# zj15001/PNP_ADMM_CNC_MRI

Measured on AMD Instinct MI355X. Metric: ADMM iterations/sec on 256x256 complex64 slices (batch=512), higher is better.
Workload: dtype f32

## Files before the change

pnp_admm_cnc_mri_amd/csrc/kernels_slice256.hip:

```cpp
#include "engine_host.h"
#include "fused_layout.h"
#include "slice_layout.h"
#include <math.h>
#include <stdio.h>
#include <stdlib.h>
#include <vector>

#ifndef SLICE_EARLY
#define SLICE_EARLY 1
#endif
#ifndef SLICE_PRIOSWAP
#define SLICE_PRIOSWAP 1
#endif
#ifndef SLICE_PRIOMASK
#define SLICE_PRIOMASK 6
#endif
#ifndef SLICE_YH_AUX
#define SLICE_YH_AUX 0
#endif
#ifndef SLICE_ST_AUX
#define SLICE_ST_AUX 0
#endif
#ifndef SLICE_PF
#define SLICE_PF 3
#endif

namespace pnp {

__device__ c32 g_tws[256];

struct SliceArgs {
    float* z;
    float* w;
    float* x;
    const c32* Yh;
    const uint32_t* Mh;
    const c32* Ys;
    const uint32_t* Ms;
    int first, B, iters;
    int slice_xor;
    int flip;
    int state_stride;
    int yh_stride;
    float scale, c;
    ProxParams prox;
    long long* prof;
};

constexpr int RP = 18;
constexpr int REGION = 16 * RP;
constexpr int WREG = 4 * REGION;
constexpr int SL_YS = SL_BUF + REGION;
constexpr int SL_LDS = SL_YS + 256 + 32;
static_assert(SL_WAVES * WREG <= SL_BUF, "wave regions must fit in the buffer they alias");

__device__ __forceinline__ void wave_sync() {
    __builtin_amdgcn_fence(__ATOMIC_RELEASE, "wavefront");
    __builtin_amdgcn_wave_barrier();
    __builtin_amdgcn_fence(__ATOMIC_ACQUIRE, "wavefront");
#ifdef SLICE_SYNC_SCHED_BARRIER
    __builtin_amdgcn_sched_barrier(0);
#endif
}

__device__ __forceinline__ void prio_set(int wv, int set) {
#if SLICE_PRIOSWAP
    const bool older_high = (SLICE_PRIOMASK >> set) & 1;
    if (set == 0 || (((SLICE_PRIOMASK >> set) ^ (SLICE_PRIOMASK >> (set - 1))) & 1)) {
        asm volatile("" : "+s"(wv));
        if ((wv < 4) == older_high) __builtin_amdgcn_s_setprio(1); else __builtin_amdgcn_s_setprio(0);
    }
#endif
}

__device__ __forceinline__ int opaque(int v) {
    asm volatile("" : "+v"(v));
    return v;
}
typedef unsigned int u32x4 __attribute__((ext_vector_type(4)));
typedef unsigned int u32x2 __attribute__((ext_vector_type(2)));
typedef __amdgpu_buffer_rsrc_t bufrsrc;
__device__ __forceinline__ bufrsrc make_rsrc(const void* base, unsigned bytes) {
    return __builtin_amdgcn_make_buffer_rsrc(const_cast<void*>(base), 0, (int)bytes, 0x00020000);
}
__device__ __forceinline__ void ld4(bufrsrc r, int voff, int soff, float (&v)[4]) {
    const u32x4 q = __builtin_amdgcn_raw_buffer_load_b128(r, voff, soff, 16);
    v[0] = __uint_as_float(q.x); v[1] = __uint_as_float(q.y); v[2] = __uint_as_float(q.z); v[3] = __uint_as_float(q.w);
}
__device__ __forceinline__ void st4(bufrsrc r, int voff, int soff, const float (&v)[4]) {
    u32x4 q;
    q.x = __float_as_uint(v[0]); q.y = __float_as_uint(v[1]); q.z = __float_as_uint(v[2]); q.w = __float_as_uint(v[3]);
    __builtin_amdgcn_raw_buffer_store_b128(q, r, voff + soff, 0, SLICE_ST_AUX);
}
__device__ __forceinline__ c32 ldc(bufrsrc r, int voff, int soff) {
    const u32x2 q = __builtin_amdgcn_raw_buffer_load_b64(r, voff, soff, 0);
    return mk<float>(__uint_as_float(q.x), __uint_as_float(q.y));
}
struct SliceBufs {
    bufrsrc z, w, x;
    bufrsrc yh, mh, ys, ms;
};

__device__ __forceinline__ void pin(c32& v) { asm volatile("" : "+v"(v.x), "+v"(v.y)); }
__device__ __forceinline__ void mem_fence_compiler() { asm volatile("" ::: "memory"); }

__device__ __forceinline__ float dpp_lane_xor1(float v) {
    return __int_as_float(__builtin_amdgcn_mov_dpp(__float_as_int(v), 0xB1 , 0xF, 0xF, true));
}
__device__ __forceinline__ c32 dpp_lane_xor1(c32 v) { return mk<float>(dpp_lane_xor1(v.x), dpp_lane_xor1(v.y)); }

__device__ __forceinline__ float sub_partner(float a, float b) {
    float r;
    asm("v_subrev_f32_dpp %0, %1, %2 quad_perm:[1,0,3,2] row_mask:0xf bank_mask:0xf bound_ctrl:1" : "=v"(r) : "v"(b), "v"(a));
    return r;
}
__device__ __forceinline__ float add_partner(float a, float b) {
    float r;
    asm("v_add_f32_dpp %0, %1, %2 quad_perm:[1,0,3,2] row_mask:0xf bank_mask:0xf bound_ctrl:1" : "=v"(r) : "v"(b), "v"(a));
    return r;
}

__device__ __forceinline__ float abs_plus(float a, float w) {
    float r;
    asm("v_add_f32_e64 %0, |%1|, %2" : "=v"(r) : "v"(a), "v"(w));
    return r;
}

__device__ __forceinline__ f2 sub2(f2 a, f2 b) {
    f2 r;
    asm("v_pk_add_f32 %0, %1, %2 neg_lo:[0,1] neg_hi:[0,1]" : "=v"(r) : "v"(a), "v"(b));
    return r;
}


template <bool INV>
__device__ __forceinline__ void group_fft256(c32 (&ac)[16], const c32* twl, c32* region, int t) {
    typedef float f4 __attribute__((ext_vector_type(4)));
    const f4* tw4 = reinterpret_cast<const f4*>(twl + RP * t);
    f2* reg2 = reinterpret_cast<f2*>(region);
    f2 a[16];
#pragma unroll
    for (int k = 0; k < 16; ++k) a[k] = to2(ac[k]);
    dft16_pk<INV>(a);
    mem_fence_compiler();
#pragma unroll
    for (int m = 0; m < 4; ++m) {
        const f4 q = tw4[m];
        if (m) a[2 * m] = tmul_v<INV>(a[2 * m], k2(q.x, q.y));
        a[2 * m + 1] = tmul_v<INV>(a[2 * m + 1], k2(q.z, q.w));
    }
    mem_fence_compiler();
#pragma unroll
    for (int m = 4; m < 8; ++m) {
        const f4 q = tw4[m];
        a[2 * m] = tmul_v<INV>(a[2 * m], k2(q.x, q.y));
        a[2 * m + 1] = tmul_v<INV>(a[2 * m + 1], k2(q.z, q.w));
    }
#pragma unroll
    for (int k = 0; k < 16; ++k) reg2[k * RP + t] = a[k];
    wave_sync();
    const f4* row4 = reinterpret_cast<const f4*>(reg2 + t * RP);
#pragma unroll
    for (int m = 0; m < 8; ++m) {
        const f4 q = row4[m];
        a[2 * m] = k2(q.x, q.y);
        a[2 * m + 1] = k2(q.z, q.w);
    }
    wave_sync();
    dft16_pk<INV>(a);
#pragma unroll
    for (int k = 0; k < 16; ++k) ac[k] = from2(a[k]);
}

struct RowLoads {
    float z[8][4], w[8][4];
};
__device__ __forceinline__ int row_set_offset(int set, int wv) { return (32 * set + 4 * wv) * 2048; }
constexpr int ROW_QSTRIDE = 256;

template <int PROX, bool HAS_INV, int Q0, int Q1>
__device__ __forceinline__ void issue_row_loads(const SliceBufs& b, RowLoads& L, int soff, int voff, int qbase = 0) {
#pragma unroll
    for (int q = qbase + Q0; q < qbase + Q1; ++q) {
        const int vo = voff + ROW_QSTRIDE * q, so = soff;
        if (PROX == 3) {
            ld4(b.w, vo, so, L.w[q]);
        } else if (PROX != 0 || !HAS_INV) {
            ld4(b.z, vo, so, L.z[q]);
            ld4(b.w, vo, so, L.w[q]);
        }
    }
}

__device__ __forceinline__ f2 clamp2(f2 a, float c) {
    return k2(__builtin_amdgcn_fmed3f(a.x, -c, c), __builtin_amdgcn_fmed3f(a.y, -c, c));
}
__device__ __forceinline__ f2 fma2(f2 a, f2 b, f2 c) { return __builtin_elementwise_fma(a, b, c); }
__device__ __forceinline__ f2 splat(float v) { return k2(v, v); }
template <int PROX>
__device__ __forceinline__ void prox_pair(f2 u, f2& z, f2& w, const ProxParams& pc) {
    if (PROX == 2) {
        const f2 cz = clamp2(z, pc.ib);
        const f2 t = fma2(splat(pc.c1), z, fma2(splat(pc.c2), u, splat(pc.c3) * cz));
        z = t - clamp2(t, pc.thr);
    } else {
        z = u - clamp2(u, pc.thr);
    }
    w = u - z;
}

template <bool HAS_INV, int PROX, bool HAS_FWD>
__device__ __forceinline__ void pointwise_q(const SliceBufs& b, const ProxParams& pc, int u_first, bool last,
                                            c32& a0, c32& a1, const float (&z_)[4], const float (&w_)[4], int vs) {
    f2 z[2] = {k2(z_[0], z_[1]), k2(z_[2], z_[3])}, w[2] = {k2(w_[0], w_[1]), k2(w_[2], w_[3])};
#define SL_X_PLUS(a_, w_) (HAS_INV ? k2(abs_plus((a_).x, (w_).x), abs_plus((a_).y, (w_).y)) : (w_))
#define SL_ST4(buf, v) { const float q_[4] = {v[0].x, v[0].y, v[1].x, v[1].y}; st4(buf, vs, 0, q_); }
    if (PROX == 3) {
        f2 u[2];
#pragma unroll
        for (int jj = 0; jj < 2; ++jj) {
            if (!u_first) {
                asm volatile("");
                w[jj] = w[jj] - (w[jj] - clamp2(w[jj], pc.thr));
            }
            u[jj] = SL_X_PLUS(jj ? a1 : a0, w[jj]);
            z[jj] = u[jj] - clamp2(u[jj], pc.thr);
            w[jj] = u[jj] - z[jj];
        }
        if (!last) {
            SL_ST4(b.w, u);
        } else {
            SL_ST4(b.z, z);
            SL_ST4(b.w, w);
        }
    }
    if (PROX == 1 || PROX == 2) {
#pragma unroll
        for (int jj = 0; jj < 2; ++jj) prox_pair<PROX>(SL_X_PLUS(jj ? a1 : a0, w[jj]), z[jj], w[jj], pc);
        SL_ST4(b.z, z);
        SL_ST4(b.w, w);
    }
#undef SL_ST4
#undef SL_X_PLUS
    if (HAS_FWD) {
        const f2 v0 = sub2(z[0], w[0]), v1 = sub2(z[1], w[1]);
        a0 = from2(v0);
        a1 = from2(v1);
    }
}

__device__ __forceinline__ void store_x_natural(const SliceBufs& b, const c32 (&a)[16], c32* wreg, int set, int wv, int lane) {
    const int g = lane >> 4, t = lane & 15;
    c32* region = wreg + g * REGION;
#pragma unroll
    for (int j = 0; j < 16; ++j) region[t + 16 * j] = mk<float>(fabsf(a[j].x), fabsf(a[j].y));
    wave_sync();
#pragma unroll
    for (int i = 0; i < 4; ++i) {
        const c32* cell = wreg + i * REGION + 4 * lane;
        const float4 c01 = *reinterpret_cast<const float4*>(cell);
        const float4 c23 = *reinterpret_cast<const float4*>(cell + 2);
        const int vs = 16 * lane + (2 * (32 * set + 4 * wv + i)) * 1024;
        const float xa[4] = {c01.x, c01.z, c23.x, c23.z}, xb[4] = {c01.y, c01.w, c23.y, c23.w};
        st4(b.x, vs, 0, xa);
        st4(b.x, vs + 1024, 0, xb);
    }
    wave_sync();
}

#ifndef SLICE_L1_PF
#define SLICE_L1_PF 8
#endif
template <int PROX> constexpr int row_pf() { return (PROX == 3) ? SLICE_L1_PF : SLICE_PF; }
template <int PROX, bool HAS_INV>
__device__ __forceinline__ void row_phase_prefetch(const SliceBufs& b, RowLoads& L, int wv, int lane) {
    issue_row_loads<PROX, HAS_INV, 0, row_pf<PROX>()>(b, L, row_set_offset(0, wv), 2048 * (lane >> 4) + 16 * (lane & 15));
}
template <bool HAS_INV, int PROX, bool HAS_FWD, bool PRELOADED = false>
__device__ __forceinline__ void row_phase(const SliceBufs& b, const ProxParams& pc, int u_first, bool last, c32 (&F)[SL_SETS][16],
                                          c32* wreg, const c32* twl, int wv, int lane, RowLoads* pre = nullptr) {
    const int g = lane >> 4, t = lane & 15;
    c32* region = wreg + g * REGION;
    const int voff = 2048 * g + 16 * t;
    constexpr int PF = row_pf<PROX>();
    RowLoads L;
    if (PRELOADED) L = *pre;
    else issue_row_loads<PROX, HAS_INV, 0, PF>(b, L, row_set_offset(0, wv), voff);
#pragma unroll
    for (int set = 0; set < SL_SETS; ++set) {
        c32 (&a)[16] = F[set];
        prio_set(wv, set);
        const int soff = row_set_offset(set, wv);
        if (HAS_INV) {
            group_fft256<true>(a, twl, region, t);
        }
        if (HAS_INV && last) store_x_natural(b, a, wreg, set, wv, lane);
        const int vs = voff + soff;
#pragma unroll
        for (int q = 0; q < 8; ++q) {
            if (q + PF < 8) issue_row_loads<PROX, HAS_INV, 0, 1>(b, L, soff, voff, q + PF);
            pointwise_q<HAS_INV, PROX, HAS_FWD>(b, pc, u_first, last, a[2 * q], a[2 * q + 1], L.z[q], L.w[q], vs + ROW_QSTRIDE * q);
        }
        if (set + 1 < SL_SETS) issue_row_loads<PROX, HAS_INV, 0, PF>(b, L, row_set_offset(set + 1, wv), voff);
        if (HAS_FWD) {
            group_fft256<false>(a, twl, region, t);
        }
    }
}

#define SL_PASS0_REGS(X, t)                                                                       \
    X(0, 0, (t)) X(1, 1, (t) + 16) X(2, 2, (t) + 32) X(3, 3, (t) + 48)                              \
    X(12, 8, ((t) ? SL_M + 64 - (t) : SL_M))                                                      \
    X(13, 13, SL_M + 48 - (t)) X(14, 14, SL_M + 32 - (t)) X(15, 15, SL_M + 16 - (t))
#define SL_PASS1_REGS(X, t)                                                                       \
    X(4, 4, (t)) X(5, 5, (t) + 16) X(6, 6, (t) + 32) X(7, 7, (t) + 48)                              \
    X(8, 12, ((t) ? SL_M + 64 - (t) : SL_M))                                                      \
    X(9, 9, SL_M + 48 - (t)) X(10, 10, SL_M + 32 - (t)) X(11, 11, SL_M + 16 - (t))

__device__ __forceinline__ void lds_put(c32* p, c32 v, bool swapped) {
    float* f = reinterpret_cast<float*>(p);
    if (swapped) { f[0] = v.y; f[1] = v.x; } else { *p = v; }
}
__device__ __forceinline__ c32 lds_get(const c32* p, bool swapped) {
    const float* f = reinterpret_cast<const float*>(p);
    return swapped ? mk<float>(f[1], f[0]) : *p;
}
template <int P>
__device__ __forceinline__ void t_store_rows(const c32 (&F)[16], c32* rp, int t) {
#define SL_T1_STORE(ja, jb, slot) { lds_put(rp + (slot), t ? F[ja] : F[jb], (ja) >= 8); }
    if (P == 0) { SL_PASS0_REGS(SL_T1_STORE, t) } else { SL_PASS1_REGS(SL_T1_STORE, t) }
#undef SL_T1_STORE
}
template <int P>
__device__ __forceinline__ void t_load_rows(c32 (&F)[16], const c32* rp, int t) {
#define SL_T2_LOAD(ja, jb, slot) { F[ja] = lds_get(rp + (slot), (ja) >= 8); }
    if (P == 0) { SL_PASS0_REGS(SL_T2_LOAD, t) } else { SL_PASS1_REGS(SL_T2_LOAD, t) }
#undef SL_T2_LOAD
    if (P == 1) {
        const c32 a0 = F[8];
        F[8] = t ? a0 : F[12];
        F[12] = t ? F[12] : a0;
    }
}

template <bool MAYBE_PACKED>
__device__ __forceinline__ void t1_read_col(c32 (&Gs)[16], const c32* buf, int off, int odd, bool packed) {
    int off_hi = off + 64 * SL_P;
    asm volatile("" : "+v"(off_hi));
    const c32 *col = buf + off, *col_hi = buf + off_hi;
#pragma unroll
    for (int jb = 0; jb < 16; jb += 8) {
        c32 own[8];
#pragma unroll
        for (int k = 0; k < 8; ++k) own[k] = jb ? col_hi[8 * k * SL_P] : col[8 * k * SL_P];
#pragma unroll
        for (int k = 0; k < 8; ++k) {
            c32 v = mk<float>(add_partner(own[k].x, own[k].y), sub_partner(own[k].y, own[k].x));
            if (MAYBE_PACKED) {
                const float oy = dpp_lane_xor1(own[k].y);
                const c32 raw = mk<float>(odd ? oy : own[k].x, odd ? own[k].x : oy);
                v = packed ? raw : v;
            }
            Gs[jb + k] = v;
            pin(Gs[jb + k]);
        }
    }
}
template <int P>
__device__ __forceinline__ void t1_pass(const c32 (&F)[SL_SETS][16], c32 (&G)[SL_SETS][16], c32* buf, int wv, int lane) {
    const int g = lane >> 4, t = lane & 15;
#pragma unroll
    for (int set = 0; set < SL_SETS; ++set) t_store_rows<P>(F[set], buf + (32 * set + 4 * wv + g) * SL_P, t);
    __syncthreads();
#pragma unroll
    for (int h = 0; h < 2; ++h) {
        const int cc = 32 * h + 4 * wv + g, odd = t & 1;
        const int off = (t >> 1) * SL_P + cc + (odd ? SL_M : 0);
        if (P == 0 && h == 0 && wv == 0) t1_read_col<true>(G[2 * P + h], buf, off, odd, cc == 0);
        else t1_read_col<false>(G[2 * P + h], buf, off, odd, false);
    }
    __syncthreads();
}

template <bool MAYBE_PACKED>
__device__ __forceinline__ void t2_write_col(const c32 (&Gs)[16], c32* buf, int off, int odd, bool packed) {
    int off_hi = off + 64 * SL_P;
    asm volatile("" : "+v"(off_hi));
    c32 *col = buf + off, *col_hi = buf + off_hi;
#pragma unroll
    for (int j = 0; j < 16; ++j) {
        const c32 own = Gs[j];
        c32 v = mk<float>(sub_partner(own.x, own.y), add_partner(own.y, own.x));
        if (MAYBE_PACKED) {
            const c32 other = dpp_lane_xor1(own);
            const c32 raw = mk<float>(odd ? own.y : own.x, odd ? other.y : other.x);
            v = packed ? raw : v;
        }
        if (j < 8) col[8 * j * SL_P] = v; else col_hi[8 * (j - 8) * SL_P] = v;
    }
}
template <int P>
__device__ __forceinline__ void t2_pass(const c32 (&G)[SL_SETS][16], c32 (&F)[SL_SETS][16], c32* buf, int wv, int lane) {
    const int g = lane >> 4, t = lane & 15;
#pragma unroll
    for (int h = 0; h < 2; ++h) {
        const int cc = 32 * h + 4 * wv + g, odd = t & 1;
        const int off = (t >> 1) * SL_P + cc + (odd ? SL_M : 0);
        if (P == 0 && h == 0 && wv == 0) t2_write_col<true>(G[2 * P + h], buf, off, odd, cc == 0);
        else t2_write_col<false>(G[2 * P + h], buf, off, odd, false);
    }
    __syncthreads();
#pragma unroll
    for (int set = 0; set < SL_SETS; ++set) t_load_rows<P>(F[set], buf + (32 * set + 4 * wv + g) * SL_P, t);
    __syncthreads();
}

struct ColLoads {
    c32 yh[16];
    uint32_t code;
};
__device__ __forceinline__ void issue_col_loads(const SliceBufs& b, ColLoads& Y, int set, int wv, int lane) {
    const int ybase = (set * 8 + wv) * 8192;
    Y.code = __builtin_amdgcn_raw_buffer_load_b32(b.mh, 4 * lane, (set * 8 + wv) * 64 * 4, 0);
#pragma unroll
    for (int jp = 0; jp < 8; ++jp) {
        const u32x4 q = __builtin_amdgcn_raw_buffer_load_b128(b.yh, 16 * lane + 1024 * (jp & 3), ybase + 4096 * (jp >> 2), SLICE_YH_AUX);
        Y.yh[2 * jp] = mk<float>(__uint_as_float(q.x), __uint_as_float(q.y));
        Y.yh[2 * jp + 1] = mk<float>(__uint_as_float(q.z), __uint_as_float(q.w));
    }
}

__device__ __forceinline__ float code_byte(unsigned m, int byte) {
    float r;
    if (byte == 0) asm("v_cvt_f32_ubyte0 %0, %1" : "=v"(r) : "v"(m));
    else if (byte == 1) asm("v_cvt_f32_ubyte1 %0, %1" : "=v"(r) : "v"(m));
    else if (byte == 2) asm("v_cvt_f32_ubyte2 %0, %1" : "=v"(r) : "v"(m));
    else asm("v_cvt_f32_ubyte3 %0, %1" : "=v"(r) : "v"(m));
    return r;
}
__device__ __forceinline__ void blend_set(c32 (&a)[16], const c32 (&yh)[16], unsigned code, float cs, float chs, float os) {
    const unsigned m[4] = {code & 0x03030303u, (code >> 2) & 0x03030303u, (code >> 4) & 0x03030303u, (code >> 6) & 0x03030303u};
#pragma unroll
    for (int j = 0; j < 16; j += 2) {
        const f2 cf = k2(code_byte(m[j & 3], j >> 2), code_byte(m[(j & 3) + 1], j >> 2));
        const f2 A2 = fma2(splat(-chs), cf, splat(os));
        a[j] = from2(fma2(A2.xx, to2(a[j]), splat(cs) * to2(yh[j])));
        a[j + 1] = from2(fma2(A2.yy, to2(a[j + 1]), splat(cs) * to2(yh[j + 1])));
    }
}

__device__ __forceinline__ void col_phase(const SliceBufs& b, float cdc, float scale, c32 (&G)[SL_SETS][16], c32* wreg, c32* ysl, const c32* twl, int wv, int lane) {
    const int g = lane >> 4, t = lane & 15;
    c32* region = wreg + g * REGION;
    const float cs = cdc * scale, chs = 0.5f * cdc * scale;
    ColLoads Y;
    issue_col_loads(b, Y, 0, wv, lane);
    if (wv == 0) {
        __builtin_amdgcn_raw_ptr_buffer_load_lds(b.ys, ysl, 16, 16 * lane, 0, 0, 0);
        __builtin_amdgcn_raw_ptr_buffer_load_lds(b.ys, ysl + 128, 16, 16 * lane, 1024, 0, 0);
        __builtin_amdgcn_raw_ptr_buffer_load_lds(b.ms, ysl + 256, 4, 4 * lane, 0, 0, 0);
    }
#pragma unroll
    for (int set = 0; set < SL_SETS; ++set) {
        c32 (&a)[16] = G[set];
        prio_set(wv, set);
        group_fft256<false>(a, twl, region, t);
        if (set == 0 && wv == 0 && g == 0) {
#pragma unroll
            for (int j = 0; j < 16; ++j) region[t + 16 * j] = a[j];
            region[256 + t] = a[0];
            wave_sync();
            const uint32_t code_b = reinterpret_cast<const uint32_t*>(ysl + 256)[t];
            const c32* mirror = region + (16 - t);
            const unsigned ma[4] = {Y.code & 0x03030303u, (Y.code >> 2) & 0x03030303u, (Y.code >> 4) & 0x03030303u, (Y.code >> 6) & 0x03030303u};
            const unsigned mb[4] = {code_b & 0x03030303u, (code_b >> 2) & 0x03030303u, (code_b >> 4) & 0x03030303u, (code_b >> 6) & 0x03030303u};
#pragma unroll
            for (int j = 0; j < 16; ++j) {
                const c32 gm = mirror[16 * (15 - j)];
                const c32 A = blend_scaled_f(unpack_a(a[j], gm), Y.yh[j], code_byte(ma[j & 3], j >> 2), cs, chs, scale);
                const c32 Bv = blend_scaled_f(unpack_b(a[j], gm), ysl[t + 16 * j], code_byte(mb[j & 3], j >> 2), cs, chs, scale);
                a[j] = repack_p(A, Bv);
            }
            wave_sync();
        } else {
            blend_set(a, Y.yh, Y.code, cs, 0.5f * chs, 0.5f * scale);
        }
        if (set + 1 < SL_SETS) issue_col_loads(b, Y, set + 1, wv, lane);
        group_fft256<true>(a, twl, region, t);
    }
}

template <int PROX>
__global__ __launch_bounds__(512) void k_slice(SliceArgs p) {
    __shared__ __attribute__((aligned(16))) c32 lds[SL_LDS];
    const int tid = threadIdx.x, lane = tid & 63;
    const int wv = __builtin_amdgcn_readfirstlane(tid >> 6);
    c32* twl = lds + SL_BUF;
    if (tid < 256) twl[RP * (tid >> 4) + (tid & 15)] = g_tws[((tid >> 4) * (tid & 15)) & 255];
    c32* wreg = lds + wv * WREG;
    __syncthreads();
    for (int sb = blockIdx.x; sb < p.B; sb += gridDim.x) {
        const int sx = ((sb ^ p.slice_xor) < p.B) ? (sb ^ p.slice_xor) : sb;
        const int slice = p.first + (p.flip ? p.B - 1 - sx : sx);
        const size_t so = (size_t)slice * p.state_stride;
        SliceBufs b;
        b.z = make_rsrc(p.z + so, 65536 * 4); b.w = make_rsrc(p.w + so, 65536 * 4); b.x = make_rsrc(p.x + (size_t)slice * 65536, 65536 * 4);
        b.yh = make_rsrc(p.Yh + (size_t)slice * p.yh_stride, YH3_SLICE * 8); b.mh = make_rsrc(p.Mh + (size_t)slice * MH3_SLICE, MH3_SLICE * 4);
        b.ys = make_rsrc(p.Ys + (size_t)slice * 256, 256 * 8); b.ms = make_rsrc(p.Ms + (size_t)slice * 16, 16 * 4);
        c32 F[SL_SETS][16];
#ifdef SLICE_PROF
        long long* prof = (p.prof && tid == 0 && sb == (int)blockIdx.x) ? p.prof + (size_t)slice * (2 + 6 * p.iters) : nullptr;
#define SL_STAMP() if (prof) *prof++ = wall_clock64()
#else
#define SL_STAMP()
#endif
        SL_STAMP();
        row_phase<false, 0, true>(b, p.prox, 1, false, F, wreg, twl, wv, opaque(lane));
        SL_STAMP();
        for (int it = 0; it < p.iters; ++it) {
            c32 G[SL_SETS][16];
            __syncthreads();
            SL_STAMP();
            t1_pass<0>(F, G, lds, wv, opaque(lane));
            t1_pass<1>(F, G, lds, wv, opaque(lane));
#ifdef SLICE_PROF_CLOCK
            if (prof) *prof++ = (long long)__builtin_readcyclecounter();
#else
            SL_STAMP();
#endif
            col_phase(b, p.c, p.scale, G, wreg, lds + SL_YS, twl, wv, opaque(lane));
            SL_STAMP();
            __syncthreads();
            SL_STAMP();
            t2_pass<0>(G, F, lds, wv, opaque(lane));
#if SLICE_EARLY
            RowLoads L0;
            row_phase_prefetch<PROX, true>(b, L0, wv, opaque(lane));
#endif
            t2_pass<1>(G, F, lds, wv, opaque(lane));
            SL_STAMP();
            const int u_first = (it == 0);
#if SLICE_EARLY
            row_phase<true, PROX, true, true>(b, p.prox, u_first, it + 1 == p.iters, F, wreg, twl, wv, opaque(lane), &L0);
#else
            row_phase<true, PROX, true>(b, p.prox, u_first, it + 1 == p.iters, F, wreg, twl, wv, opaque(lane));
#endif
            SL_STAMP();
        }
        __syncthreads();
    }
}

constexpr int SP_P = 17;
__global__ __launch_bounds__(256) void k_sprepare(const c32* y, const uint8_t* mask_bank, const int32_t* mask_id,
                                                  c32* Yh, uint32_t* Mh, c32* Ys, uint32_t* Ms, int yh_stride) {
    __shared__ c32 yd[256 * SP_P], ym[256 * SP_P];
    __shared__ uint8_t md[256 * SP_P], mm[256 * SP_P];
    const int tid = threadIdx.x, m = blockIdx.x, slice = blockIdx.y;
    const int mid = mask_id ? mask_id[slice] : 0;
    const c32* ys = y + (size_t)slice * 65536;
    const uint8_t* ms = mask_bank + (size_t)mid * 65536;
    const int ncol = (m == 8) ? 1 : 16;
#pragma unroll 4
    for (int i = 0; i < 16; ++i) {
        const int idx = tid + 256 * i, r = idx >> 4, c = idx & 15;
        if (c < ncol) {
            const int k2 = 16 * m + c, k2m = (256 - k2) & 255;
            yd[r * SP_P + c] = ys[r * 256 + k2];
            md[r * SP_P + c] = ms[r * 256 + k2];
            ym[r * SP_P + c] = ys[r * 256 + k2m];
            mm[r * SP_P + c] = ms[r * 256 + k2m];
        }
    }
    __syncthreads();
    auto entry = [&](int k1, int c, c32& yh) -> int {
        const int r2 = (256 - k1) & 255;
        const int m1 = md[k1 * SP_P + c] != 0, m2 = mm[r2 * SP_P + c] != 0;
        const c32 y1 = yd[k1 * SP_P + c], y2 = ym[r2 * SP_P + c];
        yh = mk<float>(0.5f * ((m1 ? y1.x : 0.f) + (m2 ? y2.x : 0.f)), 0.5f * ((m1 ? y1.y : 0.f) - (m2 ? y2.y : 0.f)));
        return m1 + m2;
    };
    if (m == 8) {
        c32 yh;
        const int code = entry(tid, 0, yh);
        Ys[(size_t)slice * 256 + tid] = yh;
        __shared__ int codes[256];
        codes[tid] = code;
        __syncthreads();
        if (tid < 16) {
            uint32_t v = 0;
#pragma unroll
            for (int jj = 0; jj < 16; ++jj) v |= (uint32_t)codes[tid + 16 * jj] << (2 * jj);
            Ms[slice * 16 + tid] = v;
        }
        return;
    }
    const int set = m >> 1;
#pragma unroll 4
    for (int i = 0; i < 16; ++i) {
        const int o = tid + 256 * i, blk = o >> 10, e = o & 1023;
        const int jp = e >> 7, lane = (e >> 1) & 63, j = 2 * jp + (e & 1);
        const int g = lane >> 4, t = lane & 15, wv = 4 * (m & 1) + blk;
        c32 yh;
        (void)entry(t + 16 * j, 4 * blk + g, yh);
        Yh[(size_t)slice * yh_stride + yh3_index(0, set, j, wv, lane)] = yh;
    }
    {
        const int blk = tid >> 6, lane = tid & 63, g = lane >> 4, t = lane & 15, wv = 4 * (m & 1) + blk;
        uint32_t v = 0;
#pragma unroll
        for (int j = 0; j < 16; ++j) {
            c32 yh;
            v |= (uint32_t)entry(t + 16 * j, 4 * blk + g, yh) << (2 * j);
        }
        Mh[mh3_index(slice, set, wv, lane)] = v;
    }
}

template <bool TO_SLICE>
__global__ __launch_bounds__(128) void k_state_order(const float* sz, const float* sw, float* dz, float* dw, int src_stride, int dst_stride) {
    __shared__ float tile[2][2048];
    const size_t sbase = (size_t)blockIdx.y * src_stride + (size_t)blockIdx.x * 2048, dbase = (size_t)blockIdx.y * dst_stride + (size_t)blockIdx.x * 2048;
    const float4* pz = reinterpret_cast<const float4*>(sz + sbase);
    const float4* pw = reinterpret_cast<const float4*>(sw + sbase);
    float4* qz = reinterpret_cast<float4*>(dz + dbase);
    float4* qw = reinterpret_cast<float4*>(dw + dbase);
    float4 vz[4], vw[4];
#pragma unroll
    for (int u = 0; u < 4; ++u) { vz[u] = pz[threadIdx.x + 128 * u]; vw[u] = pw[threadIdx.x + 128 * u]; }
#pragma unroll
    for (int u = 0; u < 4; ++u) {
        const int i = threadIdx.x + 128 * u, row = i >> 6, n0 = 4 * (i & 63);
        const float az[4] = {vz[u].x, vz[u].y, vz[u].z, vz[u].w}, aw[4] = {vw[u].x, vw[u].y, vw[u].z, vw[u].w};
#pragma unroll
        for (int k = 0; k < 4; ++k) {
            const int at = TO_SLICE ? (int)sl_state_index(row, n0 + k) : 4 * i + k;
            tile[0][at] = az[k];
            tile[1][at] = aw[k];
        }
    }
    __syncthreads();
#pragma unroll
    for (int u = 0; u < 4; ++u) {
        const int i = threadIdx.x + 128 * u, row = i >> 6, n0 = 4 * (i & 63);
        float oz[4], ow[4];
#pragma unroll
        for (int k = 0; k < 4; ++k) {
            const int at = TO_SLICE ? 4 * i + k : (int)sl_state_index(row, n0 + k);
            oz[k] = tile[0][at];
            ow[k] = tile[1][at];
        }
        qz[i] = make_float4(oz[0], oz[1], oz[2], oz[3]);
        qw[i] = make_float4(ow[0], ow[1], ow[2], ow[3]);
    }
}

struct Slice256 {
    int Bmax = 0, cus = 0;
    int flip = 0;
    int pad = 0, yh_pad = 0;
    float* zs = nullptr;
    float* ws = nullptr;
    c32* Yh = nullptr;
    uint32_t* Mh = nullptr;
    c32* Ys = nullptr;
    uint32_t* Ms = nullptr;
    SideQueues queues;
};

int slice256_cus(const Slice256* f) { return f && f->cus > 0 ? f->cus : 256; }

hipError_t slice256_state_order(Slice256* f, hipStream_t s, float* z, float* w, int B, bool to_slice) {
    if (B <= 0) return hipSuccess;
    if (f && f->pad > 0) {
        if (to_slice) hipLaunchKernelGGL(k_state_order<true>, dim3(32, B), dim3(128), 0, s, z, w, f->zs, f->ws, 65536, 65536 + f->pad);
        else          hipLaunchKernelGGL(k_state_order<false>, dim3(32, B), dim3(128), 0, s, f->zs, f->ws, z, w, 65536 + f->pad, 65536);
    } else {
        if (to_slice) hipLaunchKernelGGL(k_state_order<true>, dim3(32, B), dim3(128), 0, s, z, w, z, w, 65536, 65536);
        else          hipLaunchKernelGGL(k_state_order<false>, dim3(32, B), dim3(128), 0, s, z, w, z, w, 65536, 65536);
    }
    return hipGetLastError();
}

void slice256_destroy(Slice256* f) {
    if (!f) return;
    if (f->zs) (void)hipFree(f->zs);
    if (f->ws) (void)hipFree(f->ws);
    if (f->Yh) (void)hipFree(f->Yh);
    if (f->Mh) (void)hipFree(f->Mh);
    if (f->Ys) (void)hipFree(f->Ys);
    if (f->Ms) (void)hipFree(f->Ms);
    delete f;
}

Slice256* slice256_create(int Bmax, int pad_kb, int yh_pad_kb, hipError_t* err) {
    Slice256* f = new Slice256();
    f->Bmax = Bmax;
    f->pad = (pad_kb > 0 ? pad_kb : 0) * 256;
    f->yh_pad = (yh_pad_kb > 0 ? yh_pad_kb : 0) * 128;
    hipError_t e = hipMalloc((void**)&f->Yh, (size_t)Bmax * (YH3_SLICE + f->yh_pad) * sizeof(c32));
    if (e == hipSuccess && f->pad > 0) e = hipMalloc((void**)&f->zs, (size_t)Bmax * (65536 + f->pad) * sizeof(float));
// ... 96 lines not shown
```

pnp_admm_cnc_mri_amd/csrc/slice_layout.h:

```cpp
#pragma once
#include <stddef.h>
#include <stdint.h>
#include "fft16.h"

namespace pnp {

constexpr int SL_P = 132;
constexpr int SL_M = 66;
constexpr int SL_BUF = 128 * SL_P;

PNP_HD int sl_pass(int k) { return (k < 64 || k > 192 || k == 128) ? 0 : 1; }
PNP_HD int sl_slot(int k) {
    if (k < 64) return k;
    if (k == 128) return SL_M;
    if (k > 192) return SL_M + 256 - k;
    if (k < 128) return k - 64;
    return SL_M + 192 - k;
}
constexpr int SL_WAVES = 8, SL_SETS = 4;
PNP_HD int sl_unit(int set, int wv, int lane) { return 32 * set + 4 * wv + (lane >> 4); }

constexpr size_t YH3_SLICE = 4 * 16 * 8 * 64;
constexpr size_t MH3_SLICE = 4 * 8 * 64;
PNP_HD size_t yh3_index(int slice, int set, int j, int wv, int lane) {
    return (size_t)slice * YH3_SLICE + ((((size_t)set * 8 + wv) * 8 + (j >> 1)) * 64 + lane) * 2 + (j & 1);
}
PNP_HD size_t mh3_index(int slice, int set, int wv, int lane) { return (size_t)slice * MH3_SLICE + (((size_t)set * 8 + wv) * 64 + lane); }

PNP_HD size_t sl_state_index(int row, int n) {
    return (size_t)(row >> 1) * 512 + 64 * (n >> 5) + 4 * (n & 15) + 2 * ((n >> 4) & 1) + (row & 1);
}


}
```

profiles/micro/slice_stride.hip:

```cpp
#include <hip/hip_runtime.h>
#include <algorithm>
#include <cstdio>
#include <cstdlib>
#include <vector>
#define CK(x) do { hipError_t e_ = (x); if (e_ != hipSuccess) { fprintf(stderr, "%s: %s\n", #x, hipGetErrorString(e_)); exit(1); } } while (0)

__global__ __launch_bounds__(512) void k_slices(float4* z, float4* w, const float4* y, size_t stride16, int iters, int pause_ticks, long long* t, int who, int throttle) {
    if ((who == 1 && !(blockIdx.x & 1)) || (who == 2 && (blockIdx.x & 1))) { if (threadIdx.x == 0) t[blockIdx.x] = 0; return; }
    const size_t base = (size_t)blockIdx.x * stride16;
    float4* zs = z + base;
    float4* ws = w + base;
    const float4* ys = y + base;
    const int tid = threadIdx.x;
    const long long t0 = wall_clock64();
    for (int it = 0; it < iters; ++it) {
        for (int g = 0; g < 4; ++g) {
            float4 a[8], b[8], c[8];
#pragma unroll
            for (int u = 0; u < 8; ++u) { const int i = tid + 512 * (8 * g + u); a[u] = zs[i]; b[u] = ws[i]; c[u] = ys[i]; }
#pragma unroll
            for (int u = 0; u < 8; ++u) {
                const int i = tid + 512 * (8 * g + u);
                zs[i] = make_float4(a[u].x + c[u].x * 1e-9f, a[u].y + c[u].y * 1e-9f, a[u].z + c[u].z * 1e-9f, a[u].w + c[u].w * 1e-9f);
                ws[i] = make_float4(b[u].x - c[u].x * 1e-9f, b[u].y - c[u].y * 1e-9f, b[u].z - c[u].z * 1e-9f, b[u].w - c[u].w * 1e-9f);
            }
        }
        if (throttle > 0 && !(blockIdx.x & 1)) for (int k = 0; k < throttle; ++k) __builtin_amdgcn_s_sleep(24);
        if (pause_ticks > 0) {
            const long long p0 = wall_clock64();
            while (wall_clock64() - p0 < pause_ticks) __builtin_amdgcn_s_sleep(8);
        }
    }
    if (tid == 0) t[blockIdx.x] = wall_clock64() - t0;
}

int main(int argc, char** argv) {
    const size_t pad_kib = argc > 1 ? (size_t)atoi(argv[1]) : 0;
    const int slices = argc > 2 ? atoi(argv[2]) : 256;
    const int iters = argc > 3 ? atoi(argv[3]) : 50;
    const int pause_us = argc > 4 ? atoi(argv[4]) : 0;
    const int who = argc > 5 ? atoi(argv[5]) : 0, throttle = argc > 6 ? atoi(argv[6]) : 0;
    const size_t stride = (256 + pad_kib) << 10, bytes = stride * slices;
    float4 *z, *w, *y; long long* t;
    CK(hipMalloc(&z, bytes)); CK(hipMalloc(&w, bytes)); CK(hipMalloc(&y, bytes)); CK(hipMalloc(&t, slices * sizeof(long long)));
    CK(hipMemset(z, 0, bytes)); CK(hipMemset(w, 0, bytes)); CK(hipMemset(y, 0, bytes));
    hipEvent_t e0, e1; CK(hipEventCreate(&e0)); CK(hipEventCreate(&e1));
    std::vector<long long> h(slices);
    for (int rep = 0; rep < 3; ++rep) {
        CK(hipEventRecord(e0));
        hipLaunchKernelGGL(k_slices, dim3(slices), dim3(512), 0, 0, z, w, y, stride / 16, iters, pause_us * 100, t, who, throttle);
        CK(hipEventRecord(e1)); CK(hipEventSynchronize(e1));
        float ms; CK(hipEventElapsedTime(&ms, e0, e1));
        CK(hipMemcpy(h.data(), t, slices * sizeof(long long), hipMemcpyDeviceToHost));
        std::vector<double> ev, od;
        for (int b = 0; b < slices; ++b) ((b & 1) ? od : ev).push_back(h[b] / 100.0 / iters);
        std::sort(ev.begin(), ev.end()); std::sort(od.begin(), od.end());
        printf("{\"who\": %d, \"throttle\": %d, \"pad_KiB\": %zu, \"slices\": %d, \"iters\": %d, \"pause_us\": %d, \"rep\": %d, \"ms\": %.3f, \"TBps\": %.3f, "
               "\"us_per_iteration_even_median\": %.2f, \"us_per_iteration_odd_median\": %.2f, \"even_max\": %.2f, \"odd_max\": %.2f}\n",
               who, throttle, pad_kib, slices, iters, pause_us, rep, ms, 5.0 * 262144.0 * (who ? slices / 2 : slices) * iters / (ms * 1e-3) / 1e12,
               ev[ev.size() / 2], od[od.size() / 2], ev.back(), od.back());
    }
    return 0;
}
```

Baseline: 9831.

## Keep part of the w state resident in LDS and split transposes into four passes

For the PROX==2 kernel, the transpose is split into four smaller LDS passes with a narrower pitch. This frees LDS to keep the first set of w rows resident in shared memory across ADMM iterations. Those rows are read from and written to LDS instead of global memory each iteration, then flushed to global once at the end. The saving in HBM traffic costs more barrier-separated transpose passes and higher LDS occupancy per block. The microbenchmark gains a parameter that models the resident rows.

Result: faster. 10980 (median of 6 runs) (+11.7%).

```diff
diff --git a/pnp_admm_cnc_mri_amd/csrc/kernels_slice256.hip b/pnp_admm_cnc_mri_amd/csrc/kernels_slice256.hip
--- a/pnp_admm_cnc_mri_amd/csrc/kernels_slice256.hip
+++ b/pnp_admm_cnc_mri_amd/csrc/kernels_slice256.hip
@@ -20,6 +20,9 @@
 #endif
 #ifndef SLICE_ST_AUX
 #define SLICE_ST_AUX 0
+#endif
+#ifndef SLICE_RESIDENT
+#define SLICE_RESIDENT 1
 #endif
 #ifndef SLICE_PF
 #define SLICE_PF 3
@@ -53,6 +56,18 @@
 constexpr int SL_YS = SL_BUF + REGION;
 constexpr int SL_LDS = SL_YS + 256 + 32;
 static_assert(SL_WAVES * WREG <= SL_BUF, "wave regions must fit in the buffer they alias");
+constexpr int SL4_XB = SL_WAVES * WREG;
+constexpr int SL4_YS = SL4_XB + REGION;
+constexpr int SL4_RES = SL4_YS + 256 + 32;
+constexpr int SL4_LDS = SL4_RES + SL_RES * 256;
+static_assert(SL_BUF4 <= SL4_XB && SL4_RES % 2 == 0 && SL4_LDS * 8 <= 160 * 1024, "four-pass LDS map");
+template <int PROX> constexpr bool slice_four() { return PROX == 2; }
+template <int PROX> constexpr bool slice_res() { return slice_four<PROX>() && SLICE_RESIDENT; }
+__device__ __forceinline__ void lds_ld4(const float* p, float (&v)[4]) {
+    const float4 q = *reinterpret_cast<const float4*>(p);
+    v[0] = q.x; v[1] = q.y; v[2] = q.z; v[3] = q.w;
+}
+__device__ __forceinline__ void lds_st4(float* p, const float (&v)[4]) { *reinterpret_cast<float4*>(p) = make_float4(v[0], v[1], v[2], v[3]); }
 
 __device__ __forceinline__ void wave_sync() {
     __builtin_amdgcn_fence(__ATOMIC_RELEASE, "wavefront");
@@ -178,12 +193,15 @@
 __device__ __forceinline__ int row_set_offset(int set, int wv) { return (32 * set + 4 * wv) * 2048; }
 constexpr int ROW_QSTRIDE = 256;
 
-template <int PROX, bool HAS_INV, int Q0, int Q1>
-__device__ __forceinline__ void issue_row_loads(const SliceBufs& b, RowLoads& L, int soff, int voff, int qbase = 0) {
+template <int PROX, bool HAS_INV, int Q0, int Q1, bool RESW = false>
+__device__ __forceinline__ void issue_row_loads(const SliceBufs& b, RowLoads& L, int soff, int voff, int qbase = 0, const float* resw = nullptr) {
 #pragma unroll
     for (int q = qbase + Q0; q < qbase + Q1; ++q) {
         const int vo = voff + ROW_QSTRIDE * q, so = soff;
-        if (PROX == 3) {
+        if (RESW) {
+            ld4(b.z, vo, so, L.z[q]);
+            lds_ld4(resw + 64 * q, L.w[q]);
+        } else if (PROX == 3) {
             ld4(b.w, vo, so, L.w[q]);
         } else if (PROX != 0 || !HAS_INV) {
             ld4(b.z, vo, so, L.z[q]);
@@ -209,9 +227,9 @@
     w = u - z;
 }
 
-template <bool HAS_INV, int PROX, bool HAS_FWD>
+template <bool HAS_INV, int PROX, bool HAS_FWD, bool RESW = false>
 __device__ __forceinline__ void pointwise_q(const SliceBufs& b, const ProxParams& pc, int u_first, bool last,
-                                            c32& a0, c32& a1, const float (&z_)[4], const float (&w_)[4], int vs) {
+                                            c32& a0, c32& a1, const float (&z_)[4], const float (&w_)[4], int vs, float* resw = nullptr) {
     f2 z[2] = {k2(z_[0], z_[1]), k2(z_[2], z_[3])}, w[2] = {k2(w_[0], w_[1]), k2(w_[2], w_[3])};
 #define SL_X_PLUS(a_, w_) (HAS_INV ? k2(abs_plus((a_).x, (w_).x), abs_plus((a_).y, (w_).y)) : (w_))
 #define SL_ST4(buf, v) { const float q_[4] = {v[0].x, v[0].y, v[1].x, v[1].y}; st4(buf, vs, 0, q_); }
@@ -238,7 +256,8 @@
 #pragma unroll
         for (int jj = 0; jj < 2; ++jj) prox_pair<PROX>(SL_X_PLUS(jj ? a1 : a0, w[jj]), z[jj], w[jj], pc);
         SL_ST4(b.z, z);
-        SL_ST4(b.w, w);
+        if (RESW) { const float q_[4] = {w[0].x, w[0].y, w[1].x, w[1].y}; lds_st4(resw, q_); }
+        else SL_ST4(b.w, w);
     }
 #undef SL_ST4
 #undef SL_X_PLUS
@@ -272,20 +291,23 @@
 #define SLICE_L1_PF 8
 #endif
 template <int PROX> constexpr int row_pf() { return (PROX == 3) ? SLICE_L1_PF : SLICE_PF; }
-template <int PROX, bool HAS_INV>
-__device__ __forceinline__ void row_phase_prefetch(const SliceBufs& b, RowLoads& L, int wv, int lane) {
-    issue_row_loads<PROX, HAS_INV, 0, row_pf<PROX>()>(b, L, row_set_offset(0, wv), 2048 * (lane >> 4) + 16 * (lane & 15));
-}
-template <bool HAS_INV, int PROX, bool HAS_FWD, bool PRELOADED = false>
+__device__ __forceinline__ float* res_lane(float* res, int wv, int lane) { return res + sl_res_index(4 * wv + (lane >> 4), lane & 15, 0); }
+template <int PROX, bool HAS_INV, bool RES = false>
+__device__ __forceinline__ void row_phase_prefetch(const SliceBufs& b, RowLoads& L, int wv, int lane, float* res = nullptr) {
+    issue_row_loads<PROX, HAS_INV, 0, row_pf<PROX>(), RES>(b, L, row_set_offset(0, wv), 2048 * (lane >> 4) + 16 * (lane & 15), 0, RES ? res_lane(res, wv, lane) : nullptr);
+}
+template <bool HAS_INV, int PROX, bool HAS_FWD, bool PRELOADED = false, bool RES = false>
 __device__ __forceinline__ void row_phase(const SliceBufs& b, const ProxParams& pc, int u_first, bool last, c32 (&F)[SL_SETS][16],
-                                          c32* wreg, const c32* twl, int wv, int lane, RowLoads* pre = nullptr) {
+                                          c32* wreg, const c32* twl, int wv, int lane, RowLoads* pre = nullptr, float* res = nullptr) {
     const int g = lane >> 4, t = lane & 15;
     c32* region = wreg + g * REGION;
     const int voff = 2048 * g + 16 * t;
+    float* resw = RES ? res_lane(res, wv, lane) : nullptr;
+    constexpr bool RES_LOOP = RES && HAS_INV;
     constexpr int PF = row_pf<PROX>();
     RowLoads L;
     if (PRELOADED) L = *pre;
-    else issue_row_loads<PROX, HAS_INV, 0, PF>(b, L, row_set_offset(0, wv), voff);
+    else issue_row_loads<PROX, HAS_INV, 0, PF, RES_LOOP>(b, L, row_set_offset(0, wv), voff, 0, resw);
 #pragma unroll
     for (int set = 0; set < SL_SETS; ++set) {
         c32 (&a)[16] = F[set];
@@ -298,13 +320,30 @@
         const int vs = voff + soff;
 #pragma unroll
         for (int q = 0; q < 8; ++q) {
-            if (q + PF < 8) issue_row_loads<PROX, HAS_INV, 0, 1>(b, L, soff, voff, q + PF);
-            pointwise_q<HAS_INV, PROX, HAS_FWD>(b, pc, u_first, last, a[2 * q], a[2 * q + 1], L.z[q], L.w[q], vs + ROW_QSTRIDE * q);
+            if (RES_LOOP && set == 0) {
+                if (q + PF < 8) issue_row_loads<PROX, HAS_INV, 0, 1, true>(b, L, soff, voff, q + PF, resw);
+                pointwise_q<HAS_INV, PROX, HAS_FWD, true>(b, pc, u_first, last, a[2 * q], a[2 * q + 1], L.z[q], L.w[q], vs + ROW_QSTRIDE * q, resw + 64 * q);
+            } else {
+                if (q + PF < 8) issue_row_loads<PROX, HAS_INV, 0, 1>(b, L, soff, voff, q + PF);
+                if (RES && !HAS_INV && set == 0) lds_st4(resw + 64 * q, L.w[q]);
+                pointwise_q<HAS_INV, PROX, HAS_FWD>(b, pc, u_first, last, a[2 * q], a[2 * q + 1], L.z[q], L.w[q], vs + ROW_QSTRIDE * q);
+            }
         }
         if (set + 1 < SL_SETS) issue_row_loads<PROX, HAS_INV, 0, PF>(b, L, row_set_offset(set + 1, wv), voff);
         if (HAS_FWD) {
             group_fft256<false>(a, twl, region, t);
         }
+    }
+}
+
+__device__ __forceinline__ void resident_flush(const SliceBufs& b, const float* res, int wv, int lane) {
+    const float* resw = res_lane(const_cast<float*>(res), wv, lane);
+    const int vs = 2048 * (lane >> 4) + 16 * (lane & 15) + row_set_offset(0, wv);
+#pragma unroll
+    for (int q = 0; q < 8; ++q) {
+        float v[4];
+        lds_ld4(resw + 64 * q, v);
+        st4(b.w, vs + ROW_QSTRIDE * q, 0, v);
     }
 }
 
@@ -317,6 +356,11 @@
     X(8, 12, ((t) ? SL_M + 64 - (t) : SL_M))                                                      \
     X(9, 9, SL_M + 48 - (t)) X(10, 10, SL_M + 32 - (t)) X(11, 11, SL_M + 16 - (t))
 
+#define SL_PASS4_REGS(X, t, Q)                                                                    \
+    X(2 * (Q), 2 * (Q), (t)) X(2 * (Q) + 1, 2 * (Q) + 1, (t) + 16)                                  \
+    X(14 - 2 * (Q), ((Q) ? 16 - 2 * (Q) : 8), ((t) ? SL_M4 + 32 - (t) : SL_M4))                   \
+    X(15 - 2 * (Q), 15 - 2 * (Q), SL_M4 + 16 - (t))
+
 __device__ __forceinline__ void lds_put(c32* p, c32 v, bool swapped) {
     float* f = reinterpret_cast<float*>(p);
     if (swapped) { f[0] = v.y; f[1] = v.x; } else { *p = v; }
@@ -325,34 +369,41 @@
     const float* f = reinterpret_cast<const float*>(p);
     return swapped ? mk<float>(f[1], f[0]) : *p;
 }
-template <int P>
+template <int P, bool FOUR = false>
 __device__ __forceinline__ void t_store_rows(const c32 (&F)[16], c32* rp, int t) {
 #define SL_T1_STORE(ja, jb, slot) { lds_put(rp + (slot), t ? F[ja] : F[jb], (ja) >= 8); }
-    if (P == 0) { SL_PASS0_REGS(SL_T1_STORE, t) } else { SL_PASS1_REGS(SL_T1_STORE, t) }
+    if (FOUR) { SL_PASS4_REGS(SL_T1_STORE, t, P) } else if (P == 0) { SL_PASS0_REGS(SL_T1_STORE, t) } else { SL_PASS1_REGS(SL_T1_STORE, t) }
 #undef SL_T1_STORE
 }
-template <int P>
+template <int P, bool FOUR = false>
 __device__ __forceinline__ void t_load_rows(c32 (&F)[16], const c32* rp, int t) {
 #define SL_T2_LOAD(ja, jb, slot) { F[ja] = lds_get(rp + (slot), (ja) >= 8); }
-    if (P == 0) { SL_PASS0_REGS(SL_T2_LOAD, t) } else { SL_PASS1_REGS(SL_T2_LOAD, t) }
+    if (FOUR) { SL_PASS4_REGS(SL_T2_LOAD, t, P) } else if (P == 0) { SL_PASS0_REGS(SL_T2_LOAD, t) } else { SL_PASS1_REGS(SL_T2_LOAD, t) }
 #undef SL_T2_LOAD
-    if (P == 1) {
+    if (FOUR && P == 3) {
+        const c32 a8 = F[8];
+        F[8] = t ? a8 : F[14];
+        F[14] = t ? F[14] : F[12];
+        F[12] = t ? F[12] : F[10];
+        F[10] = t ? F[10] : a8;
+    }
+    if (!FOUR && P == 1) {
         const c32 a0 = F[8];
         F[8] = t ? a0 : F[12];
         F[12] = t ? F[12] : a0;
     }
 }
 
-template <bool MAYBE_PACKED>
+template <bool MAYBE_PACKED, int PITCH = SL_P>
 __device__ __forceinline__ void t1_read_col(c32 (&Gs)[16], const c32* buf, int off, int odd, bool packed) {
-    int off_hi = off + 64 * SL_P;
+    int off_hi = off + 64 * PITCH;
     asm volatile("" : "+v"(off_hi));
     const c32 *col = buf + off, *col_hi = buf + off_hi;
 #pragma unroll
     for (int jb = 0; jb < 16; jb += 8) {
         c32 own[8];
 #pragma unroll
-        for (int k = 0; k < 8; ++k) own[k] = jb ? col_hi[8 * k * SL_P] : col[8 * k * SL_P];
+        for (int k = 0; k < 8; ++k) own[k] = jb ? col_hi[8 * k * PITCH] : col[8 * k * PITCH];
 #pragma unroll
         for (int k = 0; k < 8; ++k) {
             c32 v = mk<float>(add_partner(own[k].x, own[k].y), sub_partner(own[k].y, own[k].x));
@@ -382,9 +433,9 @@
     __syncthreads();
 }
 
-template <bool MAYBE_PACKED>
+template <bool MAYBE_PACKED, int PITCH = SL_P>
 __device__ __forceinline__ void t2_write_col(const c32 (&Gs)[16], c32* buf, int off, int odd, bool packed) {
-    int off_hi = off + 64 * SL_P;
+    int off_hi = off + 64 * PITCH;
     asm volatile("" : "+v"(off_hi));
     c32 *col = buf + off, *col_hi = buf + off_hi;
 #pragma unroll
@@ -396,7 +447,7 @@
             const c32 raw = mk<float>(odd ? own.y : own.x, odd ? other.y : other.x);
             v = packed ? raw : v;
         }
-        if (j < 8) col[8 * j * SL_P] = v; else col_hi[8 * (j - 8) * SL_P] = v;
+        if (j < 8) col[8 * j * PITCH] = v; else col_hi[8 * (j - 8) * PITCH] = v;
     }
 }
 template <int P>
@@ -412,6 +463,31 @@
     __syncthreads();
 #pragma unroll
     for (int set = 0; set < SL_SETS; ++set) t_load_rows<P>(F[set], buf + (32 * set + 4 * wv + g) * SL_P, t);
+    __syncthreads();
+}
+
+template <int Q>
+__device__ __forceinline__ void t1_pass4(const c32 (&F)[SL_SETS][16], c32 (&G)[SL_SETS][16], c32* buf, int wv, int lane) {
+    const int g = lane >> 4, t = lane & 15;
+#pragma unroll
+    for (int set = 0; set < SL_SETS; ++set) t_store_rows<Q, true>(F[set], buf + (32 * set + 4 * wv + g) * SL_P4, t);
+    __syncthreads();
+    const int cc = 4 * wv + g, odd = t & 1;
+    const int off = (t >> 1) * SL_P4 + cc + (odd ? SL_M4 : 0);
+    if (Q == 0 && wv == 0) t1_read_col<true, SL_P4>(G[Q], buf, off, odd, cc == 0);
+    else t1_read_col<false, SL_P4>(G[Q], buf, off, odd, false);
+    __syncthreads();
+}
+template <int Q>
+__device__ __forceinline__ void t2_pass4(const c32 (&G)[SL_SETS][16], c32 (&F)[SL_SETS][16], c32* buf, int wv, int lane) {
+    const int g = lane >> 4, t = lane & 15;
+    const int cc = 4 * wv + g, odd = t & 1;
+    const int off = (t >> 1) * SL_P4 + cc + (odd ? SL_M4 : 0);
+    if (Q == 0 && wv == 0) t2_write_col<true, SL_P4>(G[Q], buf, off, odd, cc == 0);
+    else t2_write_col<false, SL_P4>(G[Q], buf, off, odd, false);
+    __syncthreads();
+#pragma unroll
+    for (int set = 0; set < SL_SETS; ++set) t_load_rows<Q, true>(F[set], buf + (32 * set + 4 * wv + g) * SL_P4, t);
     __syncthreads();
 }
 
@@ -492,10 +568,13 @@
 
 template <int PROX>
 __global__ __launch_bounds__(512) void k_slice(SliceArgs p) {
-    __shared__ __attribute__((aligned(16))) c32 lds[SL_LDS];
+    constexpr bool FOUR = slice_four<PROX>(), RES = slice_res<PROX>();
+    __shared__ __attribute__((aligned(16))) c32 lds[FOUR ? SL4_LDS : SL_LDS];
     const int tid = threadIdx.x, lane = tid & 63;
     const int wv = __builtin_amdgcn_readfirstlane(tid >> 6);
-    c32* twl = lds + SL_BUF;
+    c32* twl = lds + (FOUR ? SL4_XB : SL_BUF);
+    c32* ysl = lds + (FOUR ? SL4_YS : SL_YS);
+    float* res = RES ? reinterpret_cast<float*>(lds + SL4_RES) : nullptr;
     if (tid < 256) twl[RP * (tid >> 4) + (tid & 15)] = g_tws[((tid >> 4) * (tid & 15)) & 255];
     c32* wreg = lds + wv * WREG;
     __syncthreads();
@@ -515,38 +594,53 @@
 #define SL_STAMP()
 #endif
         SL_STAMP();
-        row_phase<false, 0, true>(b, p.prox, 1, false, F, wreg, twl, wv, opaque(lane));
+        row_phase<false, 0, true, false, RES>(b, p.prox, 1, false, F, wreg, twl, wv, opaque(lane), nullptr, res);
         SL_STAMP();
         for (int it = 0; it < p.iters; ++it) {
             c32 G[SL_SETS][16];
             __syncthreads();
             SL_STAMP();
-            t1_pass<0>(F, G, lds, wv, opaque(lane));
-            t1_pass<1>(F, G, lds, wv, opaque(lane));
+            if (FOUR) {
+                t1_pass4<0>(F, G, lds, wv, opaque(lane));
+                t1_pass4<1>(F, G, lds, wv, opaque(lane));
+                t1_pass4<2>(F, G, lds, wv, opaque(lane));
+                t1_pass4<3>(F, G, lds, wv, opaque(lane));
+            } else {
+                t1_pass<0>(F, G, lds, wv, opaque(lane));
+                t1_pass<1>(F, G, lds, wv, opaque(lane));
+            }
 #ifdef SLICE_PROF_CLOCK
             if (prof) *prof++ = (long long)__builtin_readcyclecounter();
 #else
             SL_STAMP();
 #endif
-            col_phase(b, p.c, p.scale, G, wreg, lds + SL_YS, twl, wv, opaque(lane));
+            col_phase(b, p.c, p.scale, G, wreg, ysl, twl, wv, opaque(lane));
             SL_STAMP();
             __syncthreads();
             SL_STAMP();
-            t2_pass<0>(G, F, lds, wv, opaque(lane));
+            if (FOUR) {
+                t2_pass4<0>(G, F, lds, wv, opaque(lane));
+                t2_pass4<1>(G, F, lds, wv, opaque(lane));
+                t2_pass4<2>(G, F, lds, wv, opaque(lane));
+            } else {
+                t2_pass<0>(G, F, lds, wv, opaque(lane));
+            }
 #if SLICE_EARLY
             RowLoads L0;
-            row_phase_prefetch<PROX, true>(b, L0, wv, opaque(lane));
-#endif
-            t2_pass<1>(G, F, lds, wv, opaque(lane));
+            row_phase_prefetch<PROX, true, RES>(b, L0, wv, opaque(lane), res);
+#endif
+            if (FOUR) t2_pass4<3>(G, F, lds, wv, opaque(lane));
+            else t2_pass<1>(G, F, lds, wv, opaque(lane));
             SL_STAMP();
             const int u_first = (it == 0);
 #if SLICE_EARLY
-            row_phase<true, PROX, true, true>(b, p.prox, u_first, it + 1 == p.iters, F, wreg, twl, wv, opaque(lane), &L0);
+            row_phase<true, PROX, true, true, RES>(b, p.prox, u_first, it + 1 == p.iters, F, wreg, twl, wv, opaque(lane), &L0, res);
 #else
-            row_phase<true, PROX, true>(b, p.prox, u_first, it + 1 == p.iters, F, wreg, twl, wv, opaque(lane));
+            row_phase<true, PROX, true, false, RES>(b, p.prox, u_first, it + 1 == p.iters, F, wreg, twl, wv, opaque(lane), nullptr, res);
 #endif
             SL_STAMP();
         }
+        if (RES) resident_flush(b, res, wv, opaque(lane));
         __syncthreads();
     }
 }
diff --git a/pnp_admm_cnc_mri_amd/csrc/slice_layout.h b/pnp_admm_cnc_mri_amd/csrc/slice_layout.h
--- a/pnp_admm_cnc_mri_amd/csrc/slice_layout.h
+++ b/pnp_admm_cnc_mri_amd/csrc/slice_layout.h
@@ -17,6 +17,14 @@
     if (k < 128) return k - 64;
     return SL_M + 192 - k;
 }
+constexpr int SL_P4 = 68;
+constexpr int SL_M4 = 34;
+constexpr int SL_BUF4 = 128 * SL_P4;
+PNP_HD int sl_pass4(int k) { return k == 128 ? 0 : k < 128 ? (k >> 5) : ((256 - k) >> 5); }
+PNP_HD int sl_slot4(int k) { return k == 128 ? SL_M4 : k < 128 ? (k & 31) : SL_M4 + ((256 - k) & 31); }
+constexpr int SL_RES = 32;
+PNP_HD int sl_res_index(int r, int t, int q) { return 512 * r + 64 * q + 4 * t; }
+
 constexpr int SL_WAVES = 8, SL_SETS = 4;
 PNP_HD int sl_unit(int set, int wv, int lane) { return 32 * set + 4 * wv + (lane >> 4); }
 
diff --git a/profiles/micro/slice_stride.hip b/profiles/micro/slice_stride.hip
--- a/profiles/micro/slice_stride.hip
+++ b/profiles/micro/slice_stride.hip
@@ -5,7 +5,7 @@
 #include <vector>
 #define CK(x) do { hipError_t e_ = (x); if (e_ != hipSuccess) { fprintf(stderr, "%s: %s\n", #x, hipGetErrorString(e_)); exit(1); } } while (0)
 
-__global__ __launch_bounds__(512) void k_slices(float4* z, float4* w, const float4* y, size_t stride16, int iters, int pause_ticks, long long* t, int who, int throttle) {
+__global__ __launch_bounds__(512) void k_slices(float4* z, float4* w, const float4* y, size_t stride16, int iters, int pause_ticks, long long* t, int who, int throttle, int res_acc) {
     if ((who == 1 && !(blockIdx.x & 1)) || (who == 2 && (blockIdx.x & 1))) { if (threadIdx.x == 0) t[blockIdx.x] = 0; return; }
     const size_t base = (size_t)blockIdx.x * stride16;
     float4* zs = z + base;
@@ -17,12 +17,12 @@
         for (int g = 0; g < 4; ++g) {
             float4 a[8], b[8], c[8];
 #pragma unroll
-            for (int u = 0; u < 8; ++u) { const int i = tid + 512 * (8 * g + u); a[u] = zs[i]; b[u] = ws[i]; c[u] = ys[i]; }
+            for (int u = 0; u < 8; ++u) { const int i = tid + 512 * (8 * g + u); a[u] = zs[i]; b[u] = (8 * g + u < res_acc) ? make_float4(0.f, 0.f, 0.f, 0.f) : ws[i]; c[u] = ys[i]; }
 #pragma unroll
             for (int u = 0; u < 8; ++u) {
                 const int i = tid + 512 * (8 * g + u);
                 zs[i] = make_float4(a[u].x + c[u].x * 1e-9f, a[u].y + c[u].y * 1e-9f, a[u].z + c[u].z * 1e-9f, a[u].w + c[u].w * 1e-9f);
-                ws[i] = make_float4(b[u].x - c[u].x * 1e-9f, b[u].y - c[u].y * 1e-9f, b[u].z - c[u].z * 1e-9f, b[u].w - c[u].w * 1e-9f);
+                if (8 * g + u >= res_acc) ws[i] = make_float4(b[u].x - c[u].x * 1e-9f, b[u].y - c[u].y * 1e-9f, b[u].z - c[u].z * 1e-9f, b[u].w - c[u].w * 1e-9f);
             }
         }
         if (throttle > 0 && !(blockIdx.x & 1)) for (int k = 0; k < throttle; ++k) __builtin_amdgcn_s_sleep(24);
@@ -40,6 +40,7 @@
     const int iters = argc > 3 ? atoi(argv[3]) : 50;
     const int pause_us = argc > 4 ? atoi(argv[4]) : 0;
     const int who = argc > 5 ? atoi(argv[5]) : 0, throttle = argc > 6 ? atoi(argv[6]) : 0;
+    const int resident = argc > 7 ? atoi(argv[7]) : 0, pause_tenths = argc > 8 ? atoi(argv[8]) : 0;
     const size_t stride = (256 + pad_kib) << 10, bytes = stride * slices;
     float4 *z, *w, *y; long long* t;
     CK(hipMalloc(&z, bytes)); CK(hipMalloc(&w, bytes)); CK(hipMalloc(&y, bytes)); CK(hipMalloc(&t, slices * sizeof(long long)));
@@ -48,16 +49,17 @@
     std::vector<long long> h(slices);
     for (int rep = 0; rep < 3; ++rep) {
         CK(hipEventRecord(e0));
-        hipLaunchKernelGGL(k_slices, dim3(slices), dim3(512), 0, 0, z, w, y, stride / 16, iters, pause_us * 100, t, who, throttle);
+        hipLaunchKernelGGL(k_slices, dim3(slices), dim3(512), 0, 0, z, w, y, stride / 16, iters, pause_us * 100 + pause_tenths * 10, t, who, throttle, resident / 4);
         CK(hipEventRecord(e1)); CK(hipEventSynchronize(e1));
         float ms; CK(hipEventElapsedTime(&ms, e0, e1));
         CK(hipMemcpy(h.data(), t, slices * sizeof(long long), hipMemcpyDeviceToHost));
         std::vector<double> ev, od;
         for (int b = 0; b < slices; ++b) ((b & 1) ? od : ev).push_back(h[b] / 100.0 / iters);
         std::sort(ev.begin(), ev.end()); std::sort(od.begin(), od.end());
-        printf("{\"who\": %d, \"throttle\": %d, \"pad_KiB\": %zu, \"slices\": %d, \"iters\": %d, \"pause_us\": %d, \"rep\": %d, \"ms\": %.3f, \"TBps\": %.3f, "
+        const double moved = (5.0 * 262144.0 - 2.0 * 2048.0 * (resident / 4 * 4)) * (who ? slices / 2 : slices) * iters;
+        printf("{\"resident\": %d, \"pause_extra_tenths\": %d, \"who\": %d, \"throttle\": %d, \"pad_KiB\": %zu, \"slices\": %d, \"iters\": %d, \"pause_us\": %d, \"rep\": %d, \"ms\": %.3f, \"TBps\": %.3f, "
                "\"us_per_iteration_even_median\": %.2f, \"us_per_iteration_odd_median\": %.2f, \"even_max\": %.2f, \"odd_max\": %.2f}\n",
-               who, throttle, pad_kib, slices, iters, pause_us, rep, ms, 5.0 * 262144.0 * (who ? slices / 2 : slices) * iters / (ms * 1e-3) / 1e12,
+               resident, pause_tenths, who, throttle, pad_kib, slices, iters, pause_us, rep, ms, moved / (ms * 1e-3) / 1e12,
                ev[ev.size() / 2], od[od.size() / 2], ev.back(), od.back());
     }
     return 0;
```
